# bentherien/point-cloud-reid

Hardware: AMD Instinct MI355X
Metric: siamese pair-comparisons/sec @1024 pts (higher is better)
Workload: dtype bf16x3

## Files before the change

### include/pcr.h

```cpp
#ifndef PCR_H_
#define PCR_H_

#ifdef __cplusplus
extern "C" {
#endif

typedef void *pcr_stream_t;

enum pcr_status {
  PCR_OK = 0,
  PCR_ERR_INVALID = 1,
  PCR_ERR_LAUNCH = 2
};

int pcr_abi_version(void);
#define PCR_PREC_F32 0
#define PCR_PREC_BF16X3 1
#define PCR_PREC_BF16 2
const char *pcr_status_string(int status);


int pcr_fps_f32(const float *xyz, float *temp, int *idx, int B, int N, int M, pcr_stream_t stream);

int pcr_fps_dist_f32(const float *dist, float *temp, int *idx, int B, int N, int M,
// ... 495 lines not shown
} pcr_attn_params;
long pcr_attn_kv_floats(int d);
int pcr_attn_kv_splits(int B, int Sk, int d);
int pcr_attn_kv_f32(const pcr_attn_params *p, pcr_stream_t stream);
int pcr_attn_apply_f32(const pcr_attn_params *p, pcr_stream_t stream);
int pcr_attn_apply_pool_ok(const pcr_attn_params *p);

typedef struct pcr_live {
  const int *count;
  int period;
  int offset;
} pcr_live;
int pcr_attn_live_ok(const pcr_attn_params *p);
int pcr_attn_kv_live_f32(const pcr_attn_params *p, const pcr_live *live, pcr_stream_t stream);
int pcr_attn_apply_live_f32(const pcr_attn_params *p, const pcr_live *live, pcr_stream_t stream);
#define PCR_ATTN_FORM_INTS 16
#define PCR_ATTN_KV_TILE 0
#define PCR_ATTN_KV_TILE_O3 1
#define PCR_ATTN_KV_TILE_O2 2
#define PCR_ATTN_KV_STREAM64 3
#define PCR_ATTN_KV_STREAM32 4
#define PCR_ATTN_KV_STREAM128 5
#define PCR_ATTN_KV_WIDE 6
#define PCR_ATTN_APPLY_TILE 7
#define PCR_ATTN_APPLY_STREAM64 8
#define PCR_ATTN_APPLY_STREAM128 9
int pcr_attn_launch_form(const pcr_attn_params *p, const pcr_live *live, int apply, int *form);

typedef struct pcr_head_params {
  int P, C, L, groups;
// ... 302 lines not shown
```

### point-cloud-reid_amd/csrc/attn_kernels_impl.h

```cpp
#pragma once
#ifndef PCR_ATTN_PREC
#define PCR_ATTN_PREC 0
#endif
#include "tile_dense.h"
#include "wave_trace.h"

#include <stdio.h>

#include <initializer_list>
#include <type_traits>
#include <vector>

namespace {
constexpr int kAPrec = PCR_ATTN_PREC;
struct AttnArgs {
  pcr_attn_params p;
  int dbg;
  int wpc;
  const int *live_count;
  int live_period, live_offset;
};

struct LiveWalk {
  unsigned n, period;
  long total;
  __device__ __forceinline__ long map(long v) const {
    const unsigned q = (unsigned)v / n;
    return (long)q * period + ((unsigned)v - q * n);
  }
};
__device__ __forceinline__ unsigned live_pairs(const AttnArgs &a) {
  int c = __builtin_amdgcn_readfirstlane(*a.live_count);
  c = c < 0 ? 0 : c;
  c -= a.live_offset;
  return (unsigned)(c < 0 ? 0 : (c > a.live_period ? a.live_period : c));
}
// ... 980 lines not shown
    const int cf = p.cfinal;
    tile_dense2p<kAPrec, TB, NR>(U, cout, p.wfinal, ceil32(cf), true, [&](float v, int o, int t) { U[o * RP + t] = v; },
                                 p.bfinal);
    __syncthreads();
    cres = cf;
  }
  float *out = p.out + b * cres * p.Lq;
  for (int e = tid; e < cres * T; e += kThreads) {
    const int c = e / T, t = e - c * T;
    if (t0 + t < p.Lq) out[(size_t)c * p.Lq + t0 + t] = U[c * RP + t];
  }
}

#if PCR_ATTN_PREC != 0
constexpr int kApsWaves = 8;
template <bool QPOS, int C1S, int CF, int NOB = 2, int ND = 2, bool POOL = false, bool GATE = false>
__global__ __launch_bounds__(64 * kApsWaves) __attribute__((amdgpu_waves_per_eu(2, 2)))
void attn_apply_stream64_kernel(AttnArgs a) {
  static_assert(!QPOS || C1S == 2 * ND, "q_pos needs c1 == d");
  static_assert(NOB <= 2 || (NOB == 4 && !CF), "cout = 128 has no trailing conv");
  static_assert(!POOL || (!CF && NOB == 2), "pooled output: cout = 64, no trailing conv");
  constexpr int D = 32 * ND, SD = 2 * ND;
  constexpr int SQ = C1S + (QPOS ? SD : 0), S0 = C1S + SD, NX = 8 * C1S;
  extern __shared__ __attribute__((aligned(16))) float smem[];
  const pcr_attn_params &p = a.p;
  bf16x8 *s_wq = reinterpret_cast<bf16x8 *>(smem);
  bf16x8 *s_w0 = s_wq + SQ * ND * 128;
  bf16x8 *s_w2 = s_w0 + S0 * ND * 256;
  float *s_c = reinterpret_cast<float *>(s_w2 + ND * NOB * 512);
  f32x4 *s_p0 = reinterpret_cast<f32x4 *>(s_c + 448);
  float *s_ks = reinterpret_cast<float *>(s_p0 + 64);
  const int tid = threadIdx.x, lane = tid & 63, j = lane & 31, h = lane >> 5;
  const int wave = __builtin_amdgcn_readfirstlane(tid >> 6);
  LiveWalk lw{};
  if constexpr (GATE) {
    lw = live_walk(a);
    if ((long)blockIdx.x * kApsWaves >= lw.total * (POOL ? 1 : (p.Lq >> 5))) return;
  }
  {
    const f32x4 *wq = reinterpret_cast<const f32x4 *>(p.wq),
                *w0 = reinterpret_cast<const f32x4 *>((p.c1 & 15) ? p.wmlp0_bf_xpad : p.wmlp0),
                *w2 = reinterpret_cast<const f32x4 *>(p.wmlp2);
    f32x4 *dq = reinterpret_cast<f32x4 *>(s_wq), *d0 = reinterpret_cast<f32x4 *>(s_w0), *d2 = reinterpret_cast<f32x4 *>(s_w2);
    for (int e = tid; e < SQ * ND * 128; e += 64 * kApsWaves) dq[e] = wq[e];
    for (int e = tid; e < S0 * ND * 256; e += 64 * kApsWaves) d0[e] = w0[e];
    for (int e = tid; e < ND * NOB * 512; e += 64 * kApsWaves) d2[e] = w2[e];
    if (tid < D) {
      s_c[tid] = p.bq[tid];
      s_c[64 + tid] = p.ln1_g[tid];
      s_c[128 + tid] = p.ln1_b[tid];

      if (QPOS) s_p0[tid] = f32x4{p.pos0_w[3 * tid], p.pos0_w[3 * tid + 1], p.pos0_w[3 * tid + 2], p.pos0_b[tid]};
// ... 16 lines not shown
  };
  auto to_ops = [&](const f32x16 &acc, int G, bf16x8 &oh, bf16x8 &ol) __attribute__((always_inline)) {
    float v[8];
#pragma unroll
    for (int e = 0; e < 8; e++) v[e] = acc[8 * G + e];
    bf_split8(v, oh, ol, true);
  };
  AttnTrace trace;
  if constexpr (kTraceBuild)
    trace.begin((a.dbg & 256) && lane == 0 && (wave == 0 || wave == 5) && blockIdx.x < kATraceWgs,
                g_attn_trace, 2 * blockIdx.x + (wave ? 1 : 0));
  const long nwav = (long)gridDim.x * kApsWaves, gw = (long)blockIdx.x * kApsWaves + wave;
  long pc = gw;
  int pblk = 0;
  float pmax = -INFINITY, psum = 0.f;
  for (long it = gw; POOL ? pc < nB : it < nitem; it += POOL ? 0 : nwav) {
    asm volatile("" ::: "memory");
    trace.mark(0);
    const long vb = POOL ? pc : it / nblk;
    const int blk = POOL ? pblk : (int)(it - vb * nblk);
    const long b = GATE ? lw.map(vb) : vb;
    const size_t bq_ = p.q_index ? (size_t)p.q_index[b] : (size_t)b;
    const size_t kb_ = p.kv_index ? (size_t)p.kv_index[b] : (size_t)b;
    const float *kvp = p.kv + kb_ * ((size_t)D * D + D);
    const int t = blk * 32 + j;
    const __amdgpu_buffer_rsrc_t rfeat = __builtin_amdgcn_make_buffer_rsrc(
        const_cast<float *>(p.feat_q + bq_ * p.c1 * p.Lq), 0, p.c1 * p.Lq * 4, 0x00020000);
    const int vo = (4 * h * p.Lq + t) * 4;
    float xf[NX];
#pragma unroll
    for (int e = 0; e < NX; e++) {
      const int ch = 16 * (e >> 3) + bf_kpos(0, e & 7);
      xf[e] = __builtin_bit_cast(float, __builtin_amdgcn_raw_buffer_load_b32(rfeat, vo, ch * p.Lq * 4, 0));
    }
// ... 244 lines not shown
        const bool up = (j & BIT) != 0;                                                               \
        _Pragma("unroll") for (int r = 0; r < N; r++) {                                               \
          const float tm = up ? vm[r + N] : vm[r], um = up ? vm[r] : vm[r + N];                       \
          const float ts = up ? vs[r + N] : vs[r], us = up ? vs[r] : vs[r + N];                       \
          vm[r] = fmaxf(tm, __uint_as_float(pcr_sort_partner<2 * J, J>(__float_as_uint(um), lane)));  \
          vs[r] = ts + __uint_as_float(pcr_sort_partner<2 * J, J>(__float_as_uint(us), lane));        \
        }                                                                                             \
      }
      PCR_POOL_STEP(8, 2, 2)
      PCR_POOL_STEP(4, 4, 4)
      PCR_POOL_STEP(2, 8, 8)
      PCR_POOL_STEP(1, 16, 16)
#undef PCR_POOL_STEP
      pmax = fmaxf(pmax, vm[0]);
      psum += vs[0];
      if (++pblk == nblk) {
        const int e = ((j & 1) << 4) | ((j & 2) << 2) | (j & 4) | ((j & 8) >> 2) | ((j & 16) >> 4);
        const int ch = 16 * (e >> 3) + bf_kpos(h, e & 7);
        float *po = p.pool_out + (size_t)b * 128;
        po[ch] = pmax;
        po[64 + ch] = psum;
        pmax = -INFINITY;
        psum = 0.f;
        pblk = 0;
        pc += nwav;
      }
    } else if constexpr (!CF) {
      const __amdgpu_buffer_rsrc_t rout =
          __builtin_amdgcn_make_buffer_rsrc(p.out + (size_t)b * (32 * NOB) * p.Lq, 0, 32 * NOB * p.Lq * 4, 0x00020000);
#pragma unroll
      for (int e = 0; e < 16 * NOB; e++) {
// ... 582 lines not shown
  return 0;
}

static void attn_dump_trace(const char *path, const char *tag, int wgs, int B, int Sk) {
  wave_trace_dump<AttnTrace>(path, HIP_SYMBOL(g_attn_trace), 2 * wgs, "kernel %s wgs %d B %d Sk %d\n", tag, wgs, B,
                             Sk);
}


struct AttnTune {
  int no_onew;
  int no_kv128;
  int kv128_wpc;
  int no_stream128;
  const char *trace;
};
static const AttnTune &attn_tune() {
  static const AttnTune once = {pcr_tune_int("PCR_ATTN_NO_ONEW"), pcr_tune_int("PCR_ATTN_NO_KV128"), pcr_tune_int("PCR_ATTN_KV128_WPC"),
                                pcr_tune_int("PCR_ATTN_NO_STREAM128"), pcr_tune_str("PCR_ATTN_TRACE")};
  return once;
}

struct AttnPlan {
  int arith = -1;
  int family = 0;
  int ntarg = 0, targ[6] = {};
  bool gated = false;
  bool trace = false;
  int threads = 0;
  size_t lds = 0;
  bool persistent = false;
  unsigned gx = 1, gy = 1;
  long work = 0;
  int per_cu = 0;
// ... 98 lines not shown
  else if (d == 128)
    rc = attn_plan_form(pl, PCR_ATTN_KV_TILE_O2, {1, 2, 1, 4, bfk && p.Sk >= 256}, false, gated);
  else rc = attn_plan_form(pl, PCR_ATTN_KV_TILE, {1, 2, 0, 4}, false, gated);
  if (rc == PCR_OK) pl->arith = PCR_PREC_F32;
  return rc;
}

static bool aps64_shape(const pcr_attn_params &p) {
  const bool aps_in = p.c1 == 64 || ((p.c1 == 32 || (p.c1 < 16 && p.wmlp0_bf_xpad)) && !p.q_pos && !p.residual);
  const bool aps_out = (p.cout == 64 && (p.cfinal == 0 || p.cfinal == 128) && p.c1 >= 32) ||
                       (p.cout == 128 && !p.cfinal && !p.residual && p.c1 == 64) ||
                       (p.cout == 32 && p.cfinal == 64 && !p.residual && p.c1 < 16);
  return p.d == 64 && aps_in && aps_out && (p.Lq & 31) == 0 && (p.nhead == 1 || p.nhead == 2 || p.nhead == 4);
}

static int attn_plan_apply(const pcr_attn_params &p, bool gated, const AttnTune &t, AttnPlan *pl) {
  (void)t;
  const int tb = p.d <= 32 ? 4 : (p.d <= 64 ? 2 : 1), T = 32 * tb, RP = T + 1;
  const int catP = ceil8(p.c1 + p.d);
  int rowsU = catP > 2 * p.d ? catP : 2 * p.d;
  if (ceil32(p.cout) > rowsU) rowsU = ceil32(p.cout);
  if (ceil32(p.cfinal) > rowsU) rowsU = ceil32(p.cfinal);
  const size_t lds = ((size_t)(rowsU + 3 + p.nhead) * RP + 2 * (kThreads / T) * T + 7 * p.d + 2 * p.cout) * sizeof(float);
  if (lds > (size_t)kMaxDynLds) return PCR_ERR_INVALID;
  pl->arith = kAPrec != 0 ? PCR_PREC_BF16X3 : PCR_PREC_F32;
#if PCR_ATTN_PREC != 0
  const long nitem = (long)p.B * (p.Lq >> 5);
  if (p.d == 128 && p.c1 == 128 && p.cout == 128 && !p.cfinal && p.q_pos && p.residual && (p.Lq & 31) == 0 && p.Lq >= 256 &&
      (p.nhead == 1 || p.nhead == 2 || p.nhead == 4) && !t.no_stream128) {
    attn_plan_persistent(pl, nitem, kAp128Waves, 1, 64 * kAp128Waves, kAp128Lds);
    return attn_plan_form(pl, PCR_ATTN_APPLY_STREAM128, {p.nhead}, false, gated);
  }
  const int aps_c1s = (p.c1 + 15) >> 4, aps_nd = p.d >> 5;
  const size_t aps_lds = (size_t)((aps_c1s + (p.q_pos ? 2 * aps_nd : 0)) * aps_nd * 128 + (aps_c1s + 2 * aps_nd) * aps_nd * 256 +
                                  aps_nd * (p.cout >> 5) * 512) * 16 +
                         (size_t)(448 + 256 + 64 * kApsWaves) * sizeof(float);
  if (p.d == 32 && p.c1 == 32 && p.cout == 32 && !p.cfinal && (p.Lq & 31) == 0 && (p.nhead == 1 || p.nhead == 2)) {
    attn_plan_persistent(pl, nitem, kApsWaves, 1, 64 * kApsWaves, aps_lds);
    return attn_plan_form(pl, PCR_ATTN_APPLY_STREAM64, {p.q_pos != 0, 2, 0, 1, 1, 0}, false, gated);
  }
  if (aps64_shape(p) && aps_lds <= (size_t)kMaxDynLds) {
    pl->trace = t.trace != nullptr;
    const int cf = p.cfinal ? 4 : 0;
    if (p.pool_out) {
      attn_plan_persistent(pl, p.B, kApsWaves, 1, 64 * kApsWaves, aps_lds);
      return attn_plan_form(pl, PCR_ATTN_APPLY_STREAM64, {0, 4, 0, 2, 2, 1}, true, gated);
    }
    attn_plan_persistent(pl, nitem, kApsWaves, 1, 64 * kApsWaves, aps_lds);
    if (p.cout == 128) return attn_plan_form(pl, PCR_ATTN_APPLY_STREAM64, {p.q_pos != 0, 4, 0, 4, 2, 0}, false, gated);
    if (p.c1 < 16) return attn_plan_form(pl, PCR_ATTN_APPLY_STREAM64, {0, 1, 2, 1, 2, 0}, false, gated);
    if (p.c1 == 32) return attn_plan_form(pl, PCR_ATTN_APPLY_STREAM64, {0, 2, cf, 2, 2, 0}, false, gated);
    return attn_plan_form(pl, PCR_ATTN_APPLY_STREAM64, {p.q_pos != 0, 4, cf, 2, 2, 0}, true, gated);
  }
#endif
  attn_plan_grid(pl, (p.Lq + T - 1) / T, p.B, lds);
  const bool wide = 2 * p.d > 128 || p.cout > 128 || p.cfinal > 128;
  if (tb == 4) return attn_plan_form(pl, PCR_ATTN_APPLY_TILE, {4, wide ? 2 : 1}, false, gated);
  if (tb == 2) return attn_plan_form(pl, PCR_ATTN_APPLY_TILE, {2, wide ? 2 : 1}, true, gated);
// ... 96 lines not shown
  }
}
#if PCR_ATTN_PREC != 0
template <bool QPOS>
static int attn_launch_apply_stream64(const AttnPlan &pl, const AttnArgs &a, const AttnTune &t, hipStream_t st) {
  const dim3 g = attn_grid(pl), blk(pl.threads);
  const int c1s = pl.targ[1], cf = pl.targ[2], nob = pl.targ[3], nd = pl.targ[4];
  int rc = PCR_ERR_INVALID;
  if (nd == 1) rc = pcr_launch_lds<attn_apply_stream64_kernel<QPOS, 2, 0, 1, 1>>(g, blk, pl.lds, st, a);
  else if (nob == 4) rc = pcr_launch_lds<attn_apply_stream64_kernel<QPOS, 4, 0, 4>>(g, blk, pl.lds, st, a);
  else if (c1s == 4 && cf && !pl.targ[5])
    rc = attn_launch_g<attn_apply_stream64_kernel<QPOS, 4, 4>, attn_apply_stream64_kernel<QPOS, 4, 4, 2, 2, false, true>>(pl, g, st, a);
  else if (c1s == 4 && !pl.targ[5])
    rc = attn_launch_g<attn_apply_stream64_kernel<QPOS, 4, 0>, attn_apply_stream64_kernel<QPOS, 4, 0, 2, 2, false, true>>(pl, g, st, a);
  else if constexpr (!QPOS) {
    if (pl.targ[5])
      return attn_launch_g<attn_apply_stream64_kernel<false, 4, 0, 2, 2, true>, attn_apply_stream64_kernel<false, 4, 0, 2, 2, true, true>>(pl, g, st, a);
    if (c1s == 1) rc = pcr_launch_lds<attn_apply_stream64_kernel<false, 1, 2, 1>>(g, blk, pl.lds, st, a);
    else if (cf) rc = pcr_launch_lds<attn_apply_stream64_kernel<false, 2, 4>>(g, blk, pl.lds, st, a);
    else rc = pcr_launch_lds<attn_apply_stream64_kernel<false, 2, 0>>(g, blk, pl.lds, st, a);
  }
  if (pl.trace) attn_dump_trace(t.trace, "apply64", (int)g.x, (int)a.p.B, a.p.Lq);
  return rc;
}
static int attn_launch_apply_stream128(const AttnPlan &pl, const AttnArgs &a, hipStream_t st) {
  const dim3 g = attn_grid(pl), blk(pl.threads);
  if (pl.targ[0] == 1) return pcr_launch_lds<attn_apply_stream128_kernel<1>>(g, blk, pl.lds, st, a);
  if (pl.targ[0] == 2) return pcr_launch_lds<attn_apply_stream128_kernel<2>>(g, blk, pl.lds, st, a);
  return pcr_launch_lds<attn_apply_stream128_kernel<4>>(g, blk, pl.lds, st, a);
}
#endif

static int attn_launch_apply(const AttnPlan &pl, const AttnArgs &a, const AttnTune &t, hipStream_t st) {
  (void)t;
  switch (pl.family) {
    case PCR_ATTN_APPLY_TILE: return attn_launch_apply_tile(pl, a, st);
#if PCR_ATTN_PREC != 0
    case PCR_ATTN_APPLY_STREAM64:
      return pl.targ[0] ? attn_launch_apply_stream64<true>(pl, a, t, st) : attn_launch_apply_stream64<false>(pl, a, t, st);
    case PCR_ATTN_APPLY_STREAM128: return attn_launch_apply_stream128(pl, a, st);
#endif
    default: return PCR_ERR_INVALID;
  }
}

static int attn_unit(const pcr_attn_params &p, const pcr_live *live, bool apply, AttnPlan *pl, bool launch, pcr_stream_t stream) {
  const AttnTune &t = attn_tune();
  *pl = AttnPlan();
  const int rc = apply ? attn_plan_apply(p, live != nullptr, t, pl) : attn_plan_kv(p, live != nullptr, t, pl);
  if (!launch) return rc;
  if (pl->arith >= 0) pcr_note_arith(pl->arith);
  if (rc != PCR_OK) return rc;
  AttnArgs a;
  a.p = p;
  a.dbg = (pl->trace ? 256 : 0) | (pcr_tune_int("PCR_ATTN_KV_FULL") ? 512 : 0);
  a.wpc = pl->wpc;
  a.live_count = live ? live->count : nullptr;
  a.live_period = live ? live->period : 0;
  a.live_offset = live ? live->offset : 0;
  return apply ? attn_launch_apply(*pl, a, t, pcr_s(stream)) : attn_launch_kv(*pl, a, t, pcr_s(stream));
}

#if PCR_ATTN_PREC == 1
int pcr_attn_kv_bf3(const pcr_attn_params *pp, const pcr_live *live, AttnPlan *pl, bool launch, pcr_stream_t stream) {
  return attn_unit(*pp, live, false, pl, launch, stream);
}
int pcr_attn_apply_bf3(const pcr_attn_params *pp, const pcr_live *live, AttnPlan *pl, bool launch, pcr_stream_t stream) {
  return attn_unit(*pp, live, true, pl, launch, stream);
}
#else
int pcr_attn_kv_bf3(const pcr_attn_params *pp, const pcr_live *live, AttnPlan *pl, bool launch, pcr_stream_t stream);
int pcr_attn_apply_bf3(const pcr_attn_params *pp, const pcr_live *live, AttnPlan *pl, bool launch, pcr_stream_t stream);

static bool attn_bf(const pcr_attn_params &p, pcr_attn_params &q) {
  const int widest = 2 * p.d > p.cout ? (2 * p.d > p.cfinal ? 2 * p.d : p.cfinal) : (p.cout > p.cfinal ? p.cout : p.cfinal);
  if (p.precision == 0 || p.d > 128 || widest > 256 || !p.wq_bf || !p.wmlp0_bf || !p.wmlp2_bf ||
      (p.cfinal && !p.wfinal_bf))
    return false;
  q = p;
  q.wq = p.wq_bf; q.wmlp0 = p.wmlp0_bf; q.wmlp2 = p.wmlp2_bf; q.wfinal = p.wfinal_bf;
  return true;
}

PCR_EXPORT int pcr_attn_kv_splits(int B, int Sk, int d) {
  (void)B;
  if (Sk < 1 || d > 64) return 1;
  if ((d == 64 || d == 32) && (Sk & 31) == 0) return 1;
  const int ntile = (Sk + 63) / 64;
  return ntile >= 16 ? 4 : (ntile >= 8 ? 2 : 1);
}

static bool attn_pool_ok(const pcr_attn_params &p) {
  pcr_attn_params q;
  return aps64_shape(p) && p.c1 == 64 && p.cout == 64 && !p.cfinal && !p.q_pos && attn_bf(p, q);
}

static int attn_entry(const pcr_attn_params *pp, const pcr_live *live, bool apply, AttnPlan *pl, bool launch, pcr_stream_t stream) {
  if (!pp || attn_check(*pp)) return PCR_ERR_INVALID;
  if (apply && ((!pp->out && !pp->pool_out) || (pp->pool_out && !attn_pool_ok(*pp)))) return PCR_ERR_INVALID;
  if (live && !attn_live_shape(*pp)) return PCR_ERR_INVALID;
  if (launch && pp->B == 0) return PCR_OK;
  if (apply && pp->B > 65535) return PCR_ERR_INVALID;
  if (live && (!live->count || live->period < 1 || live->offset < 0)) return PCR_ERR_INVALID;
  pcr_attn_params q;
  if (attn_bf(*pp, q)) return apply ? pcr_attn_apply_bf3(&q, live, pl, launch, stream) : pcr_attn_kv_bf3(&q, live, pl, launch, stream);
  return attn_unit(*pp, live, apply, pl, launch, stream);
}

PCR_EXPORT int pcr_attn_kv_f32(const pcr_attn_params *pp, pcr_stream_t stream) {
  AttnPlan pl;
  return attn_entry(pp, nullptr, false, &pl, true, stream);
}
PCR_EXPORT int pcr_attn_kv_live_f32(const pcr_attn_params *pp, const pcr_live *live, pcr_stream_t stream) {
  AttnPlan pl;
  return attn_entry(pp, live, false, &pl, true, stream);
}
PCR_EXPORT int pcr_attn_apply_f32(const pcr_attn_params *pp, pcr_stream_t stream) {
  AttnPlan pl;
  return attn_entry(pp, nullptr, true, &pl, true, stream);
}
PCR_EXPORT int pcr_attn_apply_live_f32(const pcr_attn_params *pp, const pcr_live *live, pcr_stream_t stream) {
  AttnPlan pl;
  return attn_entry(pp, live, true, &pl, true, stream);
}
PCR_EXPORT int pcr_attn_live_ok(const pcr_attn_params *pp) {
  return (pp && !attn_check(*pp) && attn_live_shape(*pp)) ? 1 : 0;
}
PCR_EXPORT int pcr_attn_apply_pool_ok(const pcr_attn_params *pp) {
  return (pp && !attn_check(*pp) && attn_pool_ok(*pp)) ? 1 : 0;
}

PCR_EXPORT int pcr_attn_launch_form(const pcr_attn_params *pp, const pcr_live *live, int apply, int *form) {
  if (!form) return PCR_ERR_INVALID;
  AttnPlan pl;
  const int rc = attn_entry(pp, live, apply != 0, &pl, false, nullptr);
  if (rc != PCR_OK) return rc;
  for (int i = 0; i < PCR_ATTN_FORM_INTS; i++) form[i] = 0;
  form[0] = pl.arith;
  form[1] = pl.family;
  form[2] = pl.gated;
  form[3] = pl.ntarg;
  for (int i = 0; i < pl.ntarg; i++) form[4 + i] = pl.targ[i];
  if (!apply) {
    form[10] = pl.splits;
    form[11] = pl.fold;
    form[12] = pl.wpc;
  }
  form[13] = (int)pl.lds;
  return PCR_OK;
}
#endif
```

### point-cloud-reid_amd/mmdet3d/models/ReIDNet.py

```python
import contextlib
import copy
from collections import OrderedDict

import torch
import torch.nn as nn

from pcr_amd import engine, frame, gallery, retrieval
from pcr_amd import _lib as L
from pcr_amd.lazylog import LazyScalars
from .attention import corss_attention, cross_lin_attn, local_self_attention
from .backbone_net import Pointnet_Backbone
from .dgcnn_orig import DGCNN
from .builder import FUSIONMODELS
from .lanegcn_nets import LinearRes
from .pointnet import PointNet
from .pointnet2_ssg import PointNet2SSG


class _OutOfScope(nn.Module):
    def __init__(self, *a, **k):
        super().__init__()
        raise NotImplementedError("%s is outside the siamese point-cloud hot path rebuilt here "
                                  "(SURVEY.md section 8f)" % type(self).__name__)

# ... 263 lines not shown
            raise ValueError("forward_inference_boxes returns (xyz, feats, lengths); ask crops_from_boxes for frames")
        clouds, lengths = crops.crops_from_boxes(points, boxes, n, **crop_args)
        if self.use_dgcnn or isinstance(self.backbone, PointNet):
            clouds = clouds.permute(0, 2, 1).contiguous()
        xyz, feats = self.forward_inference(clouds)
        return xyz, feats, lengths

    def siamese_forward(self, sparse_1, sparse_2):
        self._guard_tick(sparse_1, sparse_2)
        with self._at_level(self.precision_level()):
            return self._siamese_forward(sparse_1, sparse_2)

    def _siamese_forward(self, sparse_1, sparse_2):
        assert sparse_1.shape == sparse_2.shape
        b, num_points, _ = sparse_1.shape
        both = torch.cat([sparse_1, sparse_2], dim=0)
        if self.use_dgcnn or isinstance(self.backbone, PointNet):
            xyz, h = self.backbone(both.permute(0, 2, 1).contiguous(), self.backbone_list)
            if self.downsample is not None:
                if self.training:
                    from pcr_amd import train_graph
                    h = train_graph.downsample_points(self.downsample, h)
                else:
                    from pcr_amd import rows
                    h = rows.downsample_points(self.downsample, h)
            xyz = xyz.permute(0, 2, 1)
            return xyz[:b], xyz[b:], h[:b], h[b:]
        xyz, h = self.backbone(both, self.backbone_list)
        return xyz[:b], xyz[b:], h[:b], h[b:]

    @staticmethod
    def _pair_batch(a1, a2):
        if (a1.is_contiguous() and a2.is_contiguous() and a1.untyped_storage().data_ptr() == a2.untyped_storage().data_ptr()
                and a2.storage_offset() == a1.storage_offset() + a1.numel()):
            return a1.as_strided((2 * a1.shape[0],) + tuple(a1.shape[1:]), a1.stride(), a1.storage_offset())
        return torch.cat([a1, a2], dim=0)

    def _xcorr_eff_batched(self, h1, xyz1, h2, xyz2):
        b = h1.shape[0]
        feats = self._pair_batch(h1, h2).contiguous()
        xyz = self._pair_batch(xyz1, xyz2).contiguous()
        partner = torch.cat([torch.arange(b, 2 * b, device=feats.device, dtype=torch.int32),
                             torch.arange(0, b, device=feats.device, dtype=torch.int32)])
        s1 = self.cross_stage1.forward_paired(feats, xyz, partner)
        return self.cross_stage2.forward_paired(s1, xyz, partner)

    def xcorr_eff(self, o1, xyz1, o2, xyz2, combine="add"):
        b = o1.shape[0]
        o = self._xcorr_eff_batched(o1, xyz1, o2, xyz2)
        o1, o2 = o[:b], o[b:]
        if self.combine == "add":
            out = o1 + o2
        elif self.combine == "minus":
            out = o1 - o2
        elif self.combine == "cat":
            out = torch.cat([o1, o2], dim=1)
        elif self.combine == "point-cat":
            out = torch.cat([o1, o2], dim=2)
        else:
# ... 29 lines not shown
    def xcorr(self, search_feat, search_xyz, template_feat, template_xyz):
        a = self.cross_stage1(search_feat, search_xyz, template_feat, template_xyz)
        b = self.local_stage1(a, search_xyz)
        c = self.cross_stage2(b, search_xyz, template_feat, template_xyz)
        return self.local_stage2(c, search_xyz)

    def xcorr_baseline(self, search_feat, search_xyz, template_feat, template_xyz):
        a = self.cross_stage1(search_feat, search_xyz, template_feat, template_xyz)
        return self.cross_stage2(a, search_xyz, template_feat, template_xyz)

    def _match_logits(self, h1, h2, xyz1, xyz2, inference=False):
        if self.training:
            from pcr_amd import train_graph
            return train_graph.match_logits(self, h1, xyz1, h2, xyz2)
        if self._fused_matching():
            o = self._xcorr_eff_batched(h1, xyz1, h2, xyz2)
            return self._head(o.device).run(o), o
        if self.match_type == "xcorr_eff":
            match_in, o1, o2 = self.xcorr_eff(h1, xyz1, h2, xyz2, self.combine)
            return self._head_rows(self.get_pooled_feats(match_in)), torch.cat([o1, o2], dim=0)
        if self.match_type == "xcorr":
            if self.local_stage1 is None or self.local_stage2 is None:
                raise L.PcrError("match_type='xcorr' needs local_stage1 / local_stage2 (local_self_attention)")
            match_in = self.xcorr(h1, xyz1, h2, xyz2)
            return self._head_rows(self.get_pooled_feats(match_in)), None
        if self.match_type == "xcorr-baseline":
            match_in = self.xcorr_baseline(h1, xyz1, h2, xyz2)
            return self._head_rows(self.get_pooled_feats(match_in)), None
        if self.match_type == "concat":
            if inference:
# ... 325 lines not shown
```

### point-cloud-reid_amd/pcr_amd/abi.py

```python
import ctypes

import numpy as np
import torch

_CTYPES = {"int": ctypes.c_int, "float": ctypes.c_float, "double": ctypes.c_double, "long": ctypes.c_long}
_POINTERS = {"iptr": torch.int32, "fptr": torch.float32, "dptr": torch.float64, "lptr": torch.int64, "ptr": None}


def _block(name, decl):
    fields, elem = [], {}
    for group in decl.split(";"):
        ty, *names = group.split()
        base, _, n = ty.partition("[")
        if base in _POINTERS:
            elem.update(dict.fromkeys(names, _POINTERS[base]))
        ct = ctypes.c_void_p if base in _POINTERS else _CTYPES[base]
        fields += [(f, ct * int(n[:-1]) if n else ct) for f in names]
    return type(name, (ctypes.Structure,), {"_fields_": fields, "ELEM": elem})


def fill(p, tensors, sizes, required=(), who="pcr_amd"):
    from . import _lib as L
    elem = type(p).ELEM
    for k in tensors:
# ... 231 lines not shown
    "pcr_sa_mlp_f32": "s <SaParams>S",
    "pcr_sa_claim_ws_ints": "l iiiiii",
    "pcr_sa_tile_ws_ints": "l iiiii",
    "pcr_sa_krow_uses_tiles": "i iiiii",
    "pcr_sa_uses_row_table": "i iiiii",
    "pcr_sa_launch_form": "i <SaParams>I",
    "pcr_dense_pm_f32": "s FFFiiiiiS",
    "pcr_dense_pm_prec_f32": "s FFFiiiiiiS",
    "pcr_dense_pm_xyz_f32": "s FFFFFiiiiiiiiS",
    "pcr_sa_tables_take_xyz": "i iiiiiii",
    "pcr_attn_kv_floats": "l i",
    "pcr_attn_kv_splits": "i iii",
    "pcr_attn_kv_f32": "s <AttnParams>S",
    "pcr_attn_apply_f32": "s <AttnParams>S",
    "pcr_attn_apply_pool_ok": "i <AttnParams>",
    "pcr_attn_live_ok": "i <AttnParams>",
    "pcr_attn_kv_live_f32": "s <AttnParams><LiveParams>S",
    "pcr_attn_apply_live_f32": "s <AttnParams><LiveParams>S",
    "pcr_attn_launch_form": "i <AttnParams><LiveParams>iI",
    "pcr_pool_head_f32": "s <HeadParams>S",
    "pcr_pool_head_live_f32": "s <HeadParams><LiveParams>FS",
    "pcr_pool_both_f32": "s FFiiiS",
    "pcr_channel_max_f32": "s FFiiiiS",
    "pcr_dense_f32": "s FFFFFiiiiiS",
    "pcr_dense_xpm_f32": "s FFFFFiiiiiS",
    "pcr_dense_gn_f32": "s FFFFFFiiiiiiS",
    "pcr_dense_prec_ok": "i iii",
    "pcr_dense_prec_f32": "s FFFFFiiiiiiS",
    "pcr_dense_gn_prec_f32": "s FFFFFFiiiiiiiS",
    "pcr_dense_xpm_prec_ok": "i iii",
# ... 99 lines not shown
```

### point-cloud-reid_amd/pcr_amd/engine.py

```python
import ctypes
import os

import numpy as np
import torch

from . import _lib as L
from ._lib import _p
from .abi import AttnParams, HeadParams, LiveParams, SaParams

import os as _os
PRECISIONS = {"f32": 0, "bf16x3": 1, "bf16": 2}
PRECISION = _os.environ.get("PCR_PRECISION", "bf16x3")
if PRECISION not in PRECISIONS:
    raise L.PcrError("PCR_PRECISION must be one of %s" % sorted(PRECISIONS))


KV_SPLITS = int(os.environ["PCR_KV_SPLITS"]) if os.environ.get("PCR_KV_SPLITS") else None


def set_precision(name):
    global PRECISION
    if name not in PRECISIONS:
        raise L.PcrError("precision must be one of %s" % sorted(PRECISIONS))
    prev, PRECISION = PRECISION, name
# ... 400 lines not shown
        with _prof("attn_kv[d=%d,c2=%d,Sk=%d]" % (d, c2, Sk), kv_flops, 4.0 * B * (c2 * Sk + 3 * Sk + d * d + d),
                   arith="lib"):
            if live is not None:
                L.run.pcr_attn_kv_live_f32(ctypes.byref(p), ctypes.byref(_live_block(live)), L.stream_ptr())
            else:
                L.run.pcr_attn_kv_f32(ctypes.byref(p), L.stream_ptr())
        kv._pcr_precision = PRECISION
        return kv

    def pool_ok(self, Lq, Sk):
        dummy = torch.empty(0)
        p = self._params(1, Lq, Sk, dummy, None, dummy, None, dummy, dummy)
        p.feat_q = p.feat_k = p.xyz_k = p.kv = p.out = 1
        return bool(L.load().pcr_attn_apply_pool_ok(ctypes.byref(p)))

    def apply(self, feat_q, xyz_q, kv, Sk, kv_index=None, q_index=None, n_out=None, pooled=False, live=None, out=None):
        L.require_cuda(feat_q, kv)
        assert feat_q.is_contiguous() and feat_q.dtype == torch.float32 and (xyz_q is None or xyz_q.is_contiguous())
        Bq, c1, Lq = feat_q.shape
        assert c1 == self.c1
        made = getattr(kv, "_pcr_precision", PRECISION)
        if (made == "f32") != (PRECISION == "f32") and self.d <= 128:
            raise L.PcrError("attention state was built in %r mode and is applied in %r mode: the per-cloud matrix is "
                             "stored in the arithmetic's own layout" % (made, PRECISION))
        B = n_out if n_out is not None else Bq
        shape = (B, 2, self.cout) if pooled else (B, self.cfinal or self.cout, Lq)
        if out is not None:
            L.require_cuda(out)
            assert out.is_contiguous() and out.dtype == torch.float32 and tuple(out.shape) == shape
        if pooled:
            if out is None:
                out = (torch.zeros if live is not None else torch.empty)(shape, dtype=torch.float32, device=feat_q.device)
            p = self._params(B, Lq, Sk, feat_q, xyz_q, feat_q, xyz_q if xyz_q is not None else feat_q, kv, None,
                             kv_index, q_index)
            p.pool_out = _p(out)
        else:
            if out is None:
                out = torch.empty(shape, dtype=torch.float32, device=feat_q.device)
            p = self._params(B, Lq, Sk, feat_q, xyz_q, feat_q, xyz_q if xyz_q is not None else feat_q, kv, out,
                             kv_index, q_index)
        d = self.d
        ap_flops = 2.0 * B * Lq * (c1 * d + d * d / self.nhead + d * d + (c1 + d) * 2 * d + 2 * d * self.cout
                                   + self.cout * self.cfinal + (self.q_pos * (3 * d + d * c1)))
        with _prof("attn_apply[d=%d,c1=%d,out=%d,Lq=%d%s]" % (d, c1, self.cfinal or self.cout, Lq, ",pooled" if pooled else ""),
                   ap_flops, 4.0 * B * (c1 * Lq + d * d + d + (2 if pooled else Lq) * (self.cfinal or self.cout)), arith="lib"):
            if live is not None:
                L.run.pcr_attn_apply_live_f32(ctypes.byref(p), ctypes.byref(_live_block(live)), L.stream_ptr())
            else:
                L.run.pcr_attn_apply_f32(ctypes.byref(p), L.stream_ptr())
        return out

    def run(self, feat_q, xyz_q, feat_k, xyz_k, kv_index=None):
        assert feat_k.shape[0] == feat_q.shape[0]
        kv = self.kv(feat_k, xyz_k)
        return self.apply(feat_q, xyz_q, kv, feat_k.shape[2], kv_index=kv_index)


class HeadPlan:

    def __init__(self, linres, out_linear, device):
        if getattr(linres, "transform", None) is not None:
            raise L.PcrError("pcr_pool_head_f32 covers LinearRes with n_in == n_out only")
        L.require_default_eps(linres.norm1, linres.norm2)
        self.n = linres.linear1.weight.shape[0]
        self.groups = linres.norm1.num_groups
        self.t = dict(w1=_dev32(linres.linear1.weight, device), w2=_dev32(linres.linear2.weight, device),
                      gn1_g=_dev32(linres.norm1.weight, device), gn1_b=_dev32(linres.norm1.bias, device),
                      gn2_g=_dev32(linres.norm2.weight, device), gn2_b=_dev32(linres.norm2.bias, device),
                      w_out=_dev32(out_linear.weight, device), b_out=_dev32(out_linear.bias, device),
                      w1t=_dev32(linres.linear1.weight.detach().t().contiguous(), device),
# ... 59 lines not shown
```

Before: 67740.

## Fuse stage-2 attention with pooling via segmented partials and pair-row reduction

In inference, the siamese matching path now runs the stage-2 cross-attention in a pooled form that writes per-segment max/sum partials (8 segments per cloud, split across several waves per cloud) instead of materializing the full output. A small kernel then combines the partials for both sides of each pair into the pooled rows that feed the match head. This avoids writing and re-reading the full stage-2 feature map and raises parallelism per cloud. The partner index tensor is also cached. The cost is extra partial buffers, an additional launch, and a more complex pooling loop.

New measurement: 68090 (median of 6 runs). No clear change (+0.5%).

```diff
diff --git a/include/pcr.h b/include/pcr.h
--- a/include/pcr.h
+++ b/include/pcr.h
@@ -533,6 +533,8 @@
 int pcr_attn_live_ok(const pcr_attn_params *p);
 int pcr_attn_kv_live_f32(const pcr_attn_params *p, const pcr_live *live, pcr_stream_t stream);
 int pcr_attn_apply_live_f32(const pcr_attn_params *p, const pcr_live *live, pcr_stream_t stream);
+int pcr_attn_apply_parts_f32(const pcr_attn_params *p, const pcr_live *live, pcr_stream_t stream);
+int pcr_pool_pair_rows_f32(const float *part, float *rows, int P, int Lq, pcr_stream_t stream);
 #define PCR_ATTN_FORM_INTS 16
 #define PCR_ATTN_KV_TILE 0
 #define PCR_ATTN_KV_TILE_O3 1
diff --git a/point-cloud-reid_amd/csrc/attn_kernels_impl.h b/point-cloud-reid_amd/csrc/attn_kernels_impl.h
--- a/point-cloud-reid_amd/csrc/attn_kernels_impl.h
+++ b/point-cloud-reid_amd/csrc/attn_kernels_impl.h
@@ -20,6 +20,7 @@
   const int *live_count;
   int live_period, live_offset;
 };
+constexpr int kPoolSegs = 8;
 
 struct LiveWalk {
   unsigned n, period;
@@ -1030,12 +1031,15 @@
 
 #if PCR_ATTN_PREC != 0
 constexpr int kApsWaves = 8;
-template <bool QPOS, int C1S, int CF, int NOB = 2, int ND = 2, bool POOL = false, bool GATE = false>
+template <bool QPOS, int C1S, int CF_, int NOB = 2, int ND = 2, bool POOL = false, bool GATE = false>
 __global__ __launch_bounds__(64 * kApsWaves) __attribute__((amdgpu_waves_per_eu(2, 2)))
 void attn_apply_stream64_kernel(AttnArgs a) {
+  constexpr bool SPLIT = CF_ < 0;
+  constexpr int CF = SPLIT ? 0 : CF_;
   static_assert(!QPOS || C1S == 2 * ND, "q_pos needs c1 == d");
   static_assert(NOB <= 2 || (NOB == 4 && !CF), "cout = 128 has no trailing conv");
   static_assert(!POOL || (!CF && NOB == 2), "pooled output: cout = 64, no trailing conv");
+  static_assert(CF_ >= -1 && (!SPLIT || POOL), "CF = -1: the pooled form's partials");
   constexpr int D = 32 * ND, SD = 2 * ND;
   constexpr int SQ = C1S + (QPOS ? SD : 0), S0 = C1S + SD, NX = 8 * C1S;
   extern __shared__ __attribute__((aligned(16))) float smem[];
@@ -1051,7 +1055,7 @@
   LiveWalk lw{};
   if constexpr (GATE) {
     lw = live_walk(a);
-    if ((long)blockIdx.x * kApsWaves >= lw.total * (POOL ? 1 : (p.Lq >> 5))) return;
+    if ((long)blockIdx.x * kApsWaves >= lw.total * (POOL ? (SPLIT ? a.wpc : 1) : (p.Lq >> 5))) return;
   }
   {
     const f32x4 *wq = reinterpret_cast<const f32x4 *>(p.wq),
@@ -1098,10 +1102,40 @@
   long pc = gw;
   int pblk = 0;
   float pmax = -INFINITY, psum = 0.f;
-  for (long it = gw; POOL ? pc < nB : it < nitem; it += POOL ? 0 : nwav) {
+  const int wsh = SPLIT ? __builtin_ctz((unsigned)a.wpc) : 0, spw = kPoolSegs >> wsh;
+  const long npool = SPLIT ? nB << wsh : nB;
+  int pseg = 0;
+  auto pool_settle = [&]() __attribute__((always_inline)) {
+    while (pc < npool) {
+      if (pblk < (((pseg + 1) * nblk) >> 3)) return;
+      const long vb = pc >> wsh;
+      const long b = GATE ? lw.map(vb) : vb;
+      const int e = ((j & 1) << 4) | ((j & 2) << 2) | (j & 4) | ((j & 8) >> 2) | ((j & 16) >> 4);
+      const int ch = 16 * (e >> 3) + bf_kpos(h, e & 7);
+      float *po = p.pool_out + ((size_t)b * kPoolSegs + pseg) * 128;
+      po[ch] = pmax;
+      po[64 + ch] = psum;
+      pmax = -INFINITY;
+      psum = 0.f;
+      if ((++pseg & (spw - 1)) == 0) {
+        pc += nwav;
+        if (pc >= npool) return;
+        pseg = (int)(pc & ((1 << wsh) - 1)) * spw;
+        pblk = (pseg * nblk) >> 3;
+      }
+    }
+  };
+  if constexpr (SPLIT) {
+    if (pc < npool) {
+      pseg = (int)(pc & ((1 << wsh) - 1)) * spw;
+      pblk = (pseg * nblk) >> 3;
+      pool_settle();
+    }
+  }
+  for (long it = gw; POOL ? pc < npool : it < nitem; it += POOL ? 0 : nwav) {
     asm volatile("" ::: "memory");
     trace.mark(0);
-    const long vb = POOL ? pc : it / nblk;
+    const long vb = POOL ? (SPLIT ? pc >> wsh : pc) : it / nblk;
     const int blk = POOL ? pblk : (int)(it - vb * nblk);
     const long b = GATE ? lw.map(vb) : vb;
     const size_t bq_ = p.q_index ? (size_t)p.q_index[b] : (size_t)b;
@@ -1376,7 +1410,10 @@
 #undef PCR_POOL_STEP
       pmax = fmaxf(pmax, vm[0]);
       psum += vs[0];
-      if (++pblk == nblk) {
+      if constexpr (SPLIT) {
+        ++pblk;
+        pool_settle();
+      } else if (++pblk == nblk) {
         const int e = ((j & 1) << 4) | ((j & 2) << 2) | (j & 4) | ((j & 8) >> 2) | ((j & 16) >> 4);
         const int ch = 16 * (e >> 3) + bf_kpos(h, e & 7);
         float *po = p.pool_out + (size_t)b * 128;
@@ -1989,10 +2026,12 @@
   int kv128_wpc;
   int no_stream128;
   const char *trace;
+  int pool_wpc;
 };
 static const AttnTune &attn_tune() {
-  static const AttnTune once = {pcr_tune_int("PCR_ATTN_NO_ONEW"), pcr_tune_int("PCR_ATTN_NO_KV128"), pcr_tune_int("PCR_ATTN_KV128_WPC"),
-                                pcr_tune_int("PCR_ATTN_NO_STREAM128"), pcr_tune_str("PCR_ATTN_TRACE")};
+  static AttnTune once = {pcr_tune_int("PCR_ATTN_NO_ONEW"), pcr_tune_int("PCR_ATTN_NO_KV128"), pcr_tune_int("PCR_ATTN_KV128_WPC"),
+                          pcr_tune_int("PCR_ATTN_NO_STREAM128"), pcr_tune_str("PCR_ATTN_TRACE"), 0};
+  once.pool_wpc = pcr_tune_int("PCR_ATTN_POOL_WPC");
   return once;
 }
 
@@ -2121,7 +2160,7 @@
   return p.d == 64 && aps_in && aps_out && (p.Lq & 31) == 0 && (p.nhead == 1 || p.nhead == 2 || p.nhead == 4);
 }
 
-static int attn_plan_apply(const pcr_attn_params &p, bool gated, const AttnTune &t, AttnPlan *pl) {
+static int attn_plan_apply(const pcr_attn_params &p, bool gated, const AttnTune &t, AttnPlan *pl, bool parts) {
   (void)t;
   const int tb = p.d <= 32 ? 4 : (p.d <= 64 ? 2 : 1), T = 32 * tb, RP = T + 1;
   const int catP = ceil8(p.c1 + p.d);
@@ -2149,6 +2188,12 @@
   if (aps64_shape(p) && aps_lds <= (size_t)kMaxDynLds) {
     pl->trace = t.trace != nullptr;
     const int cf = p.cfinal ? 4 : 0;
+    if (p.pool_out && parts) {
+      const bool forced = t.pool_wpc == 1 || t.pool_wpc == 2 || t.pool_wpc == 4 || t.pool_wpc == 8;
+      pl->wpc = forced ? t.pool_wpc : attn_waves_per_cloud(p.Lq >> 5, kPoolSegs, 1);
+      attn_plan_persistent(pl, (long)p.B * pl->wpc, kApsWaves, 1, 64 * kApsWaves, aps_lds);
+      return attn_plan_form(pl, PCR_ATTN_APPLY_STREAM64, {0, 4, -1, 2, 2, 1}, true, gated);
+    }
     if (p.pool_out) {
       attn_plan_persistent(pl, p.B, kApsWaves, 1, 64 * kApsWaves, aps_lds);
       return attn_plan_form(pl, PCR_ATTN_APPLY_STREAM64, {0, 4, 0, 2, 2, 1}, true, gated);
@@ -2275,6 +2320,8 @@
   else if (c1s == 4 && !pl.targ[5])
     rc = attn_launch_g<attn_apply_stream64_kernel<QPOS, 4, 0>, attn_apply_stream64_kernel<QPOS, 4, 0, 2, 2, false, true>>(pl, g, st, a);
   else if constexpr (!QPOS) {
+    if (pl.targ[5] && cf < 0)
+      return attn_launch_g<attn_apply_stream64_kernel<false, 4, -1, 2, 2, true>, attn_apply_stream64_kernel<false, 4, -1, 2, 2, true, true>>(pl, g, st, a);
     if (pl.targ[5])
       return attn_launch_g<attn_apply_stream64_kernel<false, 4, 0, 2, 2, true>, attn_apply_stream64_kernel<false, 4, 0, 2, 2, true, true>>(pl, g, st, a);
     if (c1s == 1) rc = pcr_launch_lds<attn_apply_stream64_kernel<false, 1, 2, 1>>(g, blk, pl.lds, st, a);
@@ -2305,10 +2352,11 @@
   }
 }
 
-static int attn_unit(const pcr_attn_params &p, const pcr_live *live, bool apply, AttnPlan *pl, bool launch, pcr_stream_t stream) {
+static int attn_unit(const pcr_attn_params &p, const pcr_live *live, bool apply, AttnPlan *pl, bool launch, pcr_stream_t stream,
+                     bool parts = false) {
   const AttnTune &t = attn_tune();
   *pl = AttnPlan();
-  const int rc = apply ? attn_plan_apply(p, live != nullptr, t, pl) : attn_plan_kv(p, live != nullptr, t, pl);
+  const int rc = apply ? attn_plan_apply(p, live != nullptr, t, pl, parts) : attn_plan_kv(p, live != nullptr, t, pl);
   if (!launch) return rc;
   if (pl->arith >= 0) pcr_note_arith(pl->arith);
   if (rc != PCR_OK) return rc;
@@ -2326,12 +2374,12 @@
 int pcr_attn_kv_bf3(const pcr_attn_params *pp, const pcr_live *live, AttnPlan *pl, bool launch, pcr_stream_t stream) {
   return attn_unit(*pp, live, false, pl, launch, stream);
 }
-int pcr_attn_apply_bf3(const pcr_attn_params *pp, const pcr_live *live, AttnPlan *pl, bool launch, pcr_stream_t stream) {
-  return attn_unit(*pp, live, true, pl, launch, stream);
+int pcr_attn_apply_bf3(const pcr_attn_params *pp, const pcr_live *live, AttnPlan *pl, bool launch, pcr_stream_t stream, bool parts) {
+  return attn_unit(*pp, live, true, pl, launch, stream, parts);
 }
 #else
 int pcr_attn_kv_bf3(const pcr_attn_params *pp, const pcr_live *live, AttnPlan *pl, bool launch, pcr_stream_t stream);
-int pcr_attn_apply_bf3(const pcr_attn_params *pp, const pcr_live *live, AttnPlan *pl, bool launch, pcr_stream_t stream);
+int pcr_attn_apply_bf3(const pcr_attn_params *pp, const pcr_live *live, AttnPlan *pl, bool launch, pcr_stream_t stream, bool parts);
 
 static bool attn_bf(const pcr_attn_params &p, pcr_attn_params &q) {
   const int widest = 2 * p.d > p.cout ? (2 * p.d > p.cfinal ? 2 * p.d : p.cfinal) : (p.cout > p.cfinal ? p.cout : p.cfinal);
@@ -2356,16 +2404,18 @@
   return aps64_shape(p) && p.c1 == 64 && p.cout == 64 && !p.cfinal && !p.q_pos && attn_bf(p, q);
 }
 
-static int attn_entry(const pcr_attn_params *pp, const pcr_live *live, bool apply, AttnPlan *pl, bool launch, pcr_stream_t stream) {
+static int attn_entry(const pcr_attn_params *pp, const pcr_live *live, bool apply, AttnPlan *pl, bool launch, pcr_stream_t stream,
+                      bool parts = false) {
   if (!pp || attn_check(*pp)) return PCR_ERR_INVALID;
   if (apply && ((!pp->out && !pp->pool_out) || (pp->pool_out && !attn_pool_ok(*pp)))) return PCR_ERR_INVALID;
+  if (parts && !(apply && pp->pool_out)) return PCR_ERR_INVALID;
   if (live && !attn_live_shape(*pp)) return PCR_ERR_INVALID;
   if (launch && pp->B == 0) return PCR_OK;
   if (apply && pp->B > 65535) return PCR_ERR_INVALID;
   if (live && (!live->count || live->period < 1 || live->offset < 0)) return PCR_ERR_INVALID;
   pcr_attn_params q;
-  if (attn_bf(*pp, q)) return apply ? pcr_attn_apply_bf3(&q, live, pl, launch, stream) : pcr_attn_kv_bf3(&q, live, pl, launch, stream);
-  return attn_unit(*pp, live, apply, pl, launch, stream);
+  if (attn_bf(*pp, q)) return apply ? pcr_attn_apply_bf3(&q, live, pl, launch, stream, parts) : pcr_attn_kv_bf3(&q, live, pl, launch, stream);
+  return attn_unit(*pp, live, apply, pl, launch, stream, parts);
 }
 
 PCR_EXPORT int pcr_attn_kv_f32(const pcr_attn_params *pp, pcr_stream_t stream) {
@@ -2384,17 +2434,54 @@
   AttnPlan pl;
   return attn_entry(pp, live, true, &pl, true, stream);
 }
+PCR_EXPORT int pcr_attn_apply_parts_f32(const pcr_attn_params *pp, const pcr_live *live, pcr_stream_t stream) {
+  AttnPlan pl;
+  return attn_entry(pp, live, true, &pl, true, stream, true);
+}
 PCR_EXPORT int pcr_attn_live_ok(const pcr_attn_params *pp) {
   return (pp && !attn_check(*pp) && attn_live_shape(*pp)) ? 1 : 0;
 }
 PCR_EXPORT int pcr_attn_apply_pool_ok(const pcr_attn_params *pp) {
   return (pp && !attn_check(*pp) && attn_pool_ok(*pp)) ? 1 : 0;
+}
+
+__global__ __launch_bounds__(kThreads) void pool_pair_rows_kernel(const float *part, float *rows, int P, float n2) {
+  const int pr = (int)blockIdx.x * (kThreads / 64) + (int)(threadIdx.x >> 6);
+  const int c = threadIdx.x & 63;
+  if (pr >= P) return;
+  float mx[2], sm[2];
+#pragma unroll
+  for (int side = 0; side < 2; side++) {
+    const float *pp = part + (size_t)(pr + side * P) * (kPoolSegs * 128) + c;
+    float v[2 * kPoolSegs];
+#pragma unroll
+    for (int s = 0; s < kPoolSegs; s++) {
+      v[2 * s] = pp[s * 128];
+      v[2 * s + 1] = pp[s * 128 + 64];
+    }
+    mx[side] = -INFINITY;
+    sm[side] = 0.f;
+#pragma unroll
+    for (int s = 0; s < kPoolSegs; s++) {
+      mx[side] = fmaxf(mx[side], v[2 * s]);
+      sm[side] += v[2 * s + 1];
+    }
+  }
+  rows[(size_t)c * P + pr] = fmaxf(mx[0], mx[1]);
+  rows[(size_t)(64 + c) * P + pr] = (sm[0] + sm[1]) / n2;
+}
+PCR_EXPORT int pcr_pool_pair_rows_f32(const float *part, float *rows, int P, int Lq, pcr_stream_t stream) {
+  if (!part || !rows || P < 0 || Lq < 1) return PCR_ERR_INVALID;
+  if (P == 0) return PCR_OK;
+  const int wgs = (P + kThreads / 64 - 1) / (kThreads / 64);
+  return pcr_launch<pool_pair_rows_kernel>(dim3((unsigned)wgs), dim3(kThreads), 0, pcr_s(stream), part, rows, P,
+                                           (float)(2 * Lq));
 }
 
 PCR_EXPORT int pcr_attn_launch_form(const pcr_attn_params *pp, const pcr_live *live, int apply, int *form) {
   if (!form) return PCR_ERR_INVALID;
   AttnPlan pl;
-  const int rc = attn_entry(pp, live, apply != 0, &pl, false, nullptr);
+  const int rc = attn_entry(pp, live, apply != 0, &pl, false, nullptr, apply == 2);
   if (rc != PCR_OK) return rc;
   for (int i = 0; i < PCR_ATTN_FORM_INTS; i++) form[i] = 0;
   form[0] = pl.arith;
@@ -2405,8 +2492,8 @@
   if (!apply) {
     form[10] = pl.splits;
     form[11] = pl.fold;
-    form[12] = pl.wpc;
-  }
+  }
+  form[12] = pl.wpc;
   form[13] = (int)pl.lds;
   return PCR_OK;
 }
diff --git a/point-cloud-reid_amd/mmdet3d/models/ReIDNet.py b/point-cloud-reid_amd/mmdet3d/models/ReIDNet.py
--- a/point-cloud-reid_amd/mmdet3d/models/ReIDNet.py
+++ b/point-cloud-reid_amd/mmdet3d/models/ReIDNet.py
@@ -301,7 +301,7 @@
     def _siamese_forward(self, sparse_1, sparse_2):
         assert sparse_1.shape == sparse_2.shape
         b, num_points, _ = sparse_1.shape
-        both = torch.cat([sparse_1, sparse_2], dim=0)
+        both = self._pair_batch(sparse_1, sparse_2)
         if self.use_dgcnn or isinstance(self.backbone, PointNet):
             xyz, h = self.backbone(both.permute(0, 2, 1).contiguous(), self.backbone_list)
             if self.downsample is not None:
@@ -323,13 +323,34 @@
             return a1.as_strided((2 * a1.shape[0],) + tuple(a1.shape[1:]), a1.stride(), a1.storage_offset())
         return torch.cat([a1, a2], dim=0)
 
-    def _xcorr_eff_batched(self, h1, xyz1, h2, xyz2):
+    _PARTNER = {}
+
+    @classmethod
+    def _partner(cls, b, device):
+        key = (int(b), str(device))
+        partner = cls._PARTNER.get(key)
+        if partner is None:
+            partner = torch.cat([torch.arange(b, 2 * b, device=device, dtype=torch.int32),
+                                 torch.arange(0, b, device=device, dtype=torch.int32)])
+            if not torch.cuda.is_current_stream_capturing():
+                if len(cls._PARTNER) >= 64:
+                    cls._PARTNER.clear()
+                cls._PARTNER[key] = partner
+        return partner
+
+    def _stage2_pools(self, feats):
+        n_pts = feats.shape[2]
+        return self.cross_stage2.plan(feats.device).pool_ok(n_pts, n_pts)
+
+    def _xcorr_eff_batched(self, h1, xyz1, h2, xyz2, pooled=False):
         b = h1.shape[0]
         feats = self._pair_batch(h1, h2).contiguous()
         xyz = self._pair_batch(xyz1, xyz2).contiguous()
-        partner = torch.cat([torch.arange(b, 2 * b, device=feats.device, dtype=torch.int32),
-                             torch.arange(0, b, device=feats.device, dtype=torch.int32)])
+        partner = self._partner(b, feats.device)
         s1 = self.cross_stage1.forward_paired(feats, xyz, partner)
+        if pooled:
+            p2 = self.cross_stage2.plan(s1.device)
+            return p2.apply(s1, None, p2.kv(s1, xyz), s1.shape[2], kv_index=partner, pooled=True, parts=True)
         return self.cross_stage2.forward_paired(s1, xyz, partner)
 
     def xcorr_eff(self, o1, xyz1, o2, xyz2, combine="add"):
@@ -389,6 +410,12 @@
             from pcr_amd import train_graph
             return train_graph.match_logits(self, h1, xyz1, h2, xyz2)
         if self._fused_matching():
+            if inference and h1.shape[0] and self._stage2_pools(h1):
+                from pcr_amd import rows
+                part = self._xcorr_eff_batched(h1, xyz1, h2, xyz2, pooled=True)
+                pooled = engine.pool_pair_rows(part, h1.shape[2])
+                with engine.precision("f32"):
+                    return rows.downsample_points(self.match_head, pooled).reshape(-1), None
             o = self._xcorr_eff_batched(h1, xyz1, h2, xyz2)
             return self._head(o.device).run(o), o
         if self.match_type == "xcorr_eff":
diff --git a/point-cloud-reid_amd/pcr_amd/abi.py b/point-cloud-reid_amd/pcr_amd/abi.py
--- a/point-cloud-reid_amd/pcr_amd/abi.py
+++ b/point-cloud-reid_amd/pcr_amd/abi.py
@@ -269,6 +269,8 @@
     "pcr_attn_kv_f32": "s <AttnParams>S",
     "pcr_attn_apply_f32": "s <AttnParams>S",
     "pcr_attn_apply_pool_ok": "i <AttnParams>",
+    "pcr_attn_apply_parts_f32": "s <AttnParams><LiveParams>S",
+    "pcr_pool_pair_rows_f32": "s FFiiS",
     "pcr_attn_live_ok": "i <AttnParams>",
     "pcr_attn_kv_live_f32": "s <AttnParams><LiveParams>S",
     "pcr_attn_apply_live_f32": "s <AttnParams><LiveParams>S",
diff --git a/point-cloud-reid_amd/pcr_amd/engine.py b/point-cloud-reid_amd/pcr_amd/engine.py
--- a/point-cloud-reid_amd/pcr_amd/engine.py
+++ b/point-cloud-reid_amd/pcr_amd/engine.py
@@ -438,7 +438,8 @@
         p.feat_q = p.feat_k = p.xyz_k = p.kv = p.out = 1
         return bool(L.load().pcr_attn_apply_pool_ok(ctypes.byref(p)))
 
-    def apply(self, feat_q, xyz_q, kv, Sk, kv_index=None, q_index=None, n_out=None, pooled=False, live=None, out=None):
+    def apply(self, feat_q, xyz_q, kv, Sk, kv_index=None, q_index=None, n_out=None, pooled=False, live=None, out=None,
+              parts=False):
         L.require_cuda(feat_q, kv)
         assert feat_q.is_contiguous() and feat_q.dtype == torch.float32 and (xyz_q is None or xyz_q.is_contiguous())
         Bq, c1, Lq = feat_q.shape
@@ -448,7 +449,9 @@
             raise L.PcrError("attention state was built in %r mode and is applied in %r mode: the per-cloud matrix is "
                              "stored in the arithmetic's own layout" % (made, PRECISION))
         B = n_out if n_out is not None else Bq
-        shape = (B, 2, self.cout) if pooled else (B, self.cfinal or self.cout, Lq)
+        if parts and not pooled:
+            raise L.PcrError("apply: parts=True is a form of the pooled output")
+        shape = ((B, POOL_SEGS, 2, self.cout) if parts else (B, 2, self.cout)) if pooled else (B, self.cfinal or self.cout, Lq)
         if out is not None:
             L.require_cuda(out)
             assert out.is_contiguous() and out.dtype == torch.float32 and tuple(out.shape) == shape
@@ -468,7 +471,10 @@
                                    + self.cout * self.cfinal + (self.q_pos * (3 * d + d * c1)))
         with _prof("attn_apply[d=%d,c1=%d,out=%d,Lq=%d%s]" % (d, c1, self.cfinal or self.cout, Lq, ",pooled" if pooled else ""),
                    ap_flops, 4.0 * B * (c1 * Lq + d * d + d + (2 if pooled else Lq) * (self.cfinal or self.cout)), arith="lib"):
-            if live is not None:
+            if parts:
+                L.run.pcr_attn_apply_parts_f32(ctypes.byref(p), None if live is None else ctypes.byref(_live_block(live)),
+                                               L.stream_ptr())
+            elif live is not None:
                 L.run.pcr_attn_apply_live_f32(ctypes.byref(p), ctypes.byref(_live_block(live)), L.stream_ptr())
             else:
                 L.run.pcr_attn_apply_f32(ctypes.byref(p), L.stream_ptr())
@@ -478,6 +484,22 @@
         assert feat_k.shape[0] == feat_q.shape[0]
         kv = self.kv(feat_k, xyz_k)
         return self.apply(feat_q, xyz_q, kv, feat_k.shape[2], kv_index=kv_index)
+
+
+POOL_SEGS = 8
+
+
+def pool_pair_rows(part, Lq):
+    L.require_cuda(part)
+    if part.dtype != torch.float32 or not part.is_contiguous() or part.dim() != 4 or tuple(part.shape[1:]) != (POOL_SEGS, 2, 64) \
+            or part.shape[0] % 2:
+        raise L.PcrError("pool_pair_rows: part must be a contiguous float32 (2P, %d, 2, 64) tensor, got %s"
+                         % (POOL_SEGS, tuple(part.shape)))
+    P = part.shape[0] // 2
+    rows = torch.empty((1, 128, P), dtype=torch.float32, device=part.device)
+    with _prof("pool_pair_rows", 0.0, 4.0 * P * (2 * POOL_SEGS * 128 + 128)):
+        L.run.pcr_pool_pair_rows_f32(part, rows, P, int(Lq), L.stream_ptr())
+    return rows
 
 
 class HeadPlan:
```
